# NVIDIA/k8s-cc-manager

Measured on AMD Instinct MI355X. Metric: reconcile_gpus_per_sec, higher is better.
Workload: dtype bf16; 1 GPU; model=cc-mode-transition, global_batch=1, seq_len=1024, parallelism=concurrent-per-gpu x1, modes=on<->off toggle, device_tier=shadow+hip-attest, eviction=True, components=5, attest_gemm_dim=1024

## Files before the change

### k8s_cc_manager_amd/ops/attest_kernels.hip

```cpp

#include <hip/hip_runtime.h>
#include <hip/hip_bf16.h>

#include <cstdint>
#include <cstdio>
#include <cstdlib>
#include <mutex>

#define CC_CHECK(expr)                                                         \
  do {                                                                         \
    hipError_t _e = (expr);                                                    \
    if (_e != hipSuccess) {                                                    \
      snprintf(rep->error, sizeof(rep->error), "%s: %s", #expr,                \
               hipGetErrorString(_e));                                         \
      return (int)_e;                                                          \
    }                                                                          \
  } while (0)

using bf16 = __bf16;
typedef __attribute__((ext_vector_type(8))) bf16 bf16x8;
typedef __attribute__((ext_vector_type(4))) float f32x4;
typedef __attribute__((ext_vector_type(4))) float float4v;

constexpr int BM = 128;
constexpr int BN = 128;
constexpr int BK = 64;

__global__ void fill_bf16_lcg(bf16* __restrict__ out, long n, uint32_t seed) {
  long i = (long)blockIdx.x * blockDim.x + threadIdx.x;
  long stride = (long)gridDim.x * blockDim.x;
  for (; i < n; i += stride) {
    uint32_t x = (uint32_t)i * 1103515245u + seed * 747796405u + 12345u;
    x ^= x >> 16;
    x *= 2654435769u;
    int v = (int)((x >> 13) & 3u) - 2;
    out[i] = (bf16)(float)v;
  }
}

__global__ void fill_fp8_lcg(unsigned char* __restrict__ out, long n,
                             uint32_t seed) {
  const unsigned char enc[4] = {0xC0, 0xB8, 0x00, 0x38};
  long i = (long)blockIdx.x * blockDim.x + threadIdx.x;
  long stride = (long)gridDim.x * blockDim.x;
  for (; i < n; i += stride) {
    uint32_t x = (uint32_t)i * 1103515245u + seed * 747796405u + 12345u;
    x ^= x >> 16;
    x *= 2654435769u;
    out[i] = enc[(x >> 13) & 3u];
  }
}

constexpr int TILE_B = BM * BK * 2;

__device__ __forceinline__ int swz(int byte_off) {
  return byte_off ^ (((byte_off >> 8) & 7) << 4);
}

__device__ __forceinline__ void stage_tile_glds(
    const char* gbase, long row_stride_b, long k0_b, char* lds_tile,
    int wave, int lane) {
#pragma unroll
  for (int p = 0; p < 4; ++p) {
    int base = (wave * 4 + p) * 1024;
// ... 1304 lines not shown
}

__global__ void ref_gemm_f32(const bf16* __restrict__ A,
                             const bf16* __restrict__ Bt,
                             float* __restrict__ C, int M, int N, int K) {
  int col = blockIdx.x * blockDim.x + threadIdx.x;
  int row = blockIdx.y * blockDim.y + threadIdx.y;
  if (row >= M || col >= N) return;
  float acc = 0.f;
  const bf16* a = A + (long)row * K;
  const bf16* b = Bt + (long)col * K;
  for (int k = 0; k < K; ++k) acc = fmaf((float)a[k], (float)b[k], acc);
  C[(long)row * N + col] = acc;
}

__global__ void max_abs_diff(const float* __restrict__ x,
                             const float* __restrict__ y, long n,
                             float* out) {
  __shared__ float smax[256];
  long i = (long)blockIdx.x * blockDim.x + threadIdx.x;
  long stride = (long)gridDim.x * blockDim.x;
  float m = 0.f;
  for (; i < n; i += stride) {
    float d = fabsf(x[i] - y[i]);
    m = fmaxf(m, d);
  }
  smax[threadIdx.x] = m;
  __syncthreads();
  for (int s = 128; s > 0; s >>= 1) {
    if (threadIdx.x < s) smax[threadIdx.x] = fmaxf(smax[threadIdx.x], smax[threadIdx.x + s]);
    __syncthreads();
  }
  if (threadIdx.x == 0) {
    atomicMax((unsigned int*)out, __float_as_uint(smax[0]));
  }
}

__global__ void checksum_f32(const float* __restrict__ x, long n,
                             unsigned long long* out) {
  long i = (long)blockIdx.x * blockDim.x + threadIdx.x;
  long stride = (long)gridDim.x * blockDim.x;
  unsigned long long h = 0;
  for (; i < n; i += stride) {
    unsigned long long v = (unsigned long long)__float_as_uint(x[i]) + 0x9e3779b97f4a7c15ull * (unsigned long long)(i + 1);
    v ^= v >> 33; v *= 0xff51afd7ed558ccdull; v ^= v >> 33;
    h ^= v;
  }
  for (int off = 32; off > 0; off >>= 1)
    h ^= __shfl_down(h, off, 64);
  __shared__ unsigned long long partial[4];
  if ((threadIdx.x & 63) == 0) partial[threadIdx.x >> 6] = h;
  __syncthreads();
  if (threadIdx.x == 0) {
    unsigned long long b = partial[0];
    for (int w = 1; w < (int)(blockDim.x >> 6); ++w) b ^= partial[w];
    atomicXor(out, b);
  }
}

constexpr int LDS_PROBE_WORDS = 16384;

__global__ void lds_probe(uint32_t* __restrict__ fail_count, int rounds) {
  __shared__ uint32_t slab[LDS_PROBE_WORDS];
  const int tid = threadIdx.x;
  const int nthreads = blockDim.x;
  uint32_t local_fail = 0;
  for (int r = 0; r < rounds; ++r) {
    uint32_t salt = 0x9e3779b9u * (r + 1) + blockIdx.x;
    for (int i = tid; i < LDS_PROBE_WORDS; i += nthreads)
      slab[i] = (uint32_t)i * 2654435769u + salt;
    __syncthreads();
    for (int i = tid; i < LDS_PROBE_WORDS; i += nthreads) {
// ... 3 lines not shown
    }
    __syncthreads();
  }
  if (local_fail) atomicAdd(fail_count, local_fail);
}

__global__ void hbm_copy_f4(const float4v* __restrict__ src,
                            float4v* __restrict__ dst, long n4) {
  long i = (long)blockIdx.x * blockDim.x + threadIdx.x;
  long stride = (long)gridDim.x * blockDim.x;
  for (; i < n4; i += stride) dst[i] = src[i];
}

constexpr int kMaxDevices = 64;

struct ProbeCtx {
  int dim = 0;
  int ref_valid = 0;
  bf16 *dA = nullptr, *dB = nullptr;
  unsigned char *dA8 = nullptr, *dB8 = nullptr;
  float *dC = nullptr, *dRef = nullptr, *dHbm = nullptr, *dErr = nullptr;
  unsigned long long* dSum = nullptr;
  uint32_t* dFail = nullptr;
  int* dLive = nullptr;
  hipEvent_t ev0 = nullptr, ev1 = nullptr;
  float* dPeerDst = nullptr;
  long peer_cap = 0;
  unsigned long long* dPeerSum = nullptr;
  int peer_cursor = 0;
};

static ProbeCtx g_ctx[kMaxDevices];
static std::mutex g_ctx_mu;

static void ctx_release(ProbeCtx& c) {
  if (c.dA) (void)hipFree(c.dA);
  if (c.dB) (void)hipFree(c.dB);
  if (c.dA8) (void)hipFree(c.dA8);
  if (c.dB8) (void)hipFree(c.dB8);
  if (c.dC) (void)hipFree(c.dC);
  if (c.dRef) (void)hipFree(c.dRef);
  if (c.dHbm) (void)hipFree(c.dHbm);
  if (c.dErr) (void)hipFree(c.dErr);
  if (c.dSum) (void)hipFree(c.dSum);
  if (c.dFail) (void)hipFree(c.dFail);
  if (c.dLive) (void)hipFree(c.dLive);
  if (c.dPeerDst) (void)hipFree(c.dPeerDst);
  if (c.dPeerSum) (void)hipFree(c.dPeerSum);
  if (c.ev0) (void)hipEventDestroy(c.ev0);
  if (c.ev1) (void)hipEventDestroy(c.ev1);
  c = ProbeCtx{};
}

static hipError_t ctx_acquire(int device, int dim, ProbeCtx** out) {
  ProbeCtx& c = g_ctx[device];
  if (c.dim == dim) {
    *out = &c;
    return hipSuccess;
  }
  ctx_release(c);
  long elems = (long)dim * dim;
  hipError_t e;
  if ((e = hipMalloc(&c.dA, elems * sizeof(bf16))) != hipSuccess) return e;
  if ((e = hipMalloc(&c.dB, elems * sizeof(bf16))) != hipSuccess) return e;
  if ((e = hipMalloc(&c.dA8, elems)) != hipSuccess) return e;
  if ((e = hipMalloc(&c.dB8, elems)) != hipSuccess) return e;
  if ((e = hipMalloc(&c.dC, elems * sizeof(float))) != hipSuccess) return e;
  if ((e = hipMalloc(&c.dRef, elems * sizeof(float))) != hipSuccess) return e;
  if ((e = hipMalloc(&c.dHbm, elems * sizeof(float))) != hipSuccess) return e;
  if ((e = hipMalloc(&c.dErr, sizeof(float))) != hipSuccess) return e;
  if ((e = hipMalloc(&c.dSum, sizeof(unsigned long long))) != hipSuccess) return e;
  if ((e = hipMalloc(&c.dFail, sizeof(uint32_t))) != hipSuccess) return e;
  if ((e = hipMalloc(&c.dLive, sizeof(int))) != hipSuccess) return e;
  if ((e = hipEventCreate(&c.ev0)) != hipSuccess) return e;
  if ((e = hipEventCreate(&c.ev1)) != hipSuccess) return e;
  c.dim = dim;
  *out = &c;
  return hipSuccess;
}


extern "C" {

struct CcAttestReport {
  int device;
  int cu_count;
  int xcc_count;
  char arch[64];
  char error[256];
  long long vram_total_mb;
// ... 15 lines not shown
  int peers_attempted;
  int peers_verified;
  double xgmi_ms;
  double xgmi_gbps_min;
  double xgmi_gbps_max;
  int ok;
};

__global__ void liveness_kernel(int* out) {
  if (threadIdx.x == 0 && blockIdx.x == 0) *out = 0x600D;
}

int cc_device_alive(int device) {
  if (device < 0 || device >= kMaxDevices) return -1;
  if (hipSetDevice(device) != hipSuccess) return -1;
  int* d = nullptr;
  {
    std::lock_guard<std::mutex> lk(g_ctx_mu);
    ProbeCtx& c = g_ctx[device];
    if (!c.dLive && hipMalloc(&c.dLive, sizeof(int)) != hipSuccess) return -2;
    d = c.dLive;
  }
  if (hipMemset(d, 0, sizeof(int)) != hipSuccess) return -2;
  hipLaunchKernelGGL(liveness_kernel, dim3(1), dim3(64), 0, 0, d);
  int h = 0;
  hipError_t e = hipMemcpy(&h, d, sizeof(int), hipMemcpyDeviceToHost);
  if (e != hipSuccess) return -3;
  return h == 0x600D ? 0 : -4;
}

int cc_device_count(void) {
  int n = 0;
  if (hipGetDeviceCount(&n) != hipSuccess) return -1;
  return n;
}

int cc_device_index_for_bdf(int domain, int bus, int dev) {
  int n = 0;
  if (hipGetDeviceCount(&n) != hipSuccess) return -1;
  for (int i = 0; i < n; ++i) {
    hipDeviceProp_t p;
    if (hipGetDeviceProperties(&p, i) != hipSuccess) continue;
    if (p.pciDomainID == domain && p.pciBusID == bus && p.pciDeviceID == dev)
      return i;
  }
  return -1;
}

static int launch_mfma_gemm(const void* A, const void* Bt, void* C, int M,
                            int N, int K) {
  if (M % BM == 0 && N % BN == 0 && K % BK == 0 &&
      ((long)(N / BN) * (M / BM)) <= 256) {
    dim3 grid(N / BN, M / BM);
    hipLaunchKernelGGL(mfma_gemm_bf16, grid, dim3(256), 0, 0, (const bf16*)A,
                       (const bf16*)Bt, (float*)C, M, N, K);
    return 0;
  }
  if (M % BM2 == 0 && N % BN2 == 0 && K % (2 * BK2) == 0) {
    dim3 grid(N / BN2, M / BM2);
    long ws = 2L * K * (M + N) + 4L * M * N;
    int swz_on = ws > (256L << 20) ? 1 : 0;
    if ((long)grid.x * grid.y <= 256)
      hipLaunchKernelGGL(mfma_gemm_bf16_256w, grid, dim3(512), 0, 0,
                         (const bf16*)A, (const bf16*)Bt, (float*)C, M, N, K,
                         swz_on);
    else
      hipLaunchKernelGGL(mfma_gemm_bf16_256, grid, dim3(512), 0, 0,
                         (const bf16*)A, (const bf16*)Bt, (float*)C, M, N, K,
                         swz_on);
    return 0;
  }
  if (M % BM || N % BN || K % BK) return -2;
  dim3 grid(N / BN, M / BM);
  hipLaunchKernelGGL(mfma_gemm_bf16, grid, dim3(256), 0, 0, (const bf16*)A,
                     (const bf16*)Bt, (float*)C, M, N, K);
  return 0;
}

int cc_mfma_gemm_bf16(int device, const void* A, const void* Bt, void* C,
                      int M, int N, int K) {
  if (hipSetDevice(device) != hipSuccess) return -3;
  int rc = launch_mfma_gemm(A, Bt, C, M, N, K);
  if (rc != 0) return rc;
  return (int)hipDeviceSynchronize();
}

int cc_mfma_gemm_bf16_variant(int device, const void* A, const void* Bt,
                              void* C, int M, int N, int K, int which) {
  if (hipSetDevice(device) != hipSuccess) return -3;
// ... 88 lines not shown
    dim3 grid(N / BN2, M / BM2);
    long ws = (long)K * (M + N) + 4L * M * N;
    hipLaunchKernelGGL(mfma_gemm_fp8_256, grid, dim3(512), 0, 0,
                       (const char*)A, (const char*)Bt, (float*)C, M, N, K,
                       ws > (256L << 20) ? 1 : 0);
  } else {
    if (M % BM || N % BN || K % BK8) return -2;
    dim3 grid(N / BN, M / BM);
    hipLaunchKernelGGL(mfma_gemm_fp8_128, grid, dim3(256), 0, 0,
                       (const char*)A, (const char*)Bt, (float*)C, M, N, K);
  }
  return (int)hipDeviceSynchronize();
}

static int launch_fp8_best(const void* A, const void* Bt, void* C, int M,
                           int N, int K) {
  if (M % BM || N % BN) return -2;
  dim3 grid(N / BN, M / BM);
  long ws = (long)K * (M + N) + 4L * M * N;
  int swz_on = ws > (256L << 20) ? 1 : 0;
  if (K % BK8 == 0) {
    long blocks = (long)grid.x * grid.y;
    if (blocks <= 256)
      hipLaunchKernelGGL(mfma_gemm_fp8_128pc, grid, dim3(512), 0, 0,
                         (const char*)A, (const char*)Bt, (float*)C, M, N, K,
                         swz_on);
    else
      hipLaunchKernelGGL(mfma_gemm_fp8_128u, grid, dim3(256), 0, 0,
                         (const char*)A, (const char*)Bt, (float*)C, M, N, K,
                         swz_on);
    return 0;
  }
  if (K % 64 == 0) {
    hipLaunchKernelGGL(mfma_gemm_fp8_128s, grid, dim3(256), 0, 0,
                       (const char*)A, (const char*)Bt, (float*)C, M, N, K);
    return 0;
  }
  return -2;
}

int cc_mfma_gemm_fp8(int device, const void* A, const void* Bt, void* C,
                     int M, int N, int K) {
  if (hipSetDevice(device) != hipSuccess) return -3;
  int rc = launch_fp8_best(A, Bt, C, M, N, K);
  if (rc != 0) return rc;
  return (int)hipDeviceSynchronize();
}

int cc_ref_gemm_f32(int device, const void* A, const void* Bt, void* C,
                    int M, int N, int K) {
  if (hipSetDevice(device) != hipSuccess) return -3;
  dim3 block(16, 16);
  dim3 grid((N + 15) / 16, (M + 15) / 16);
  hipLaunchKernelGGL(ref_gemm_f32, grid, block, 0, 0, (const bf16*)A,
                     (const bf16*)Bt, (float*)C, M, N, K);
  return (int)hipDeviceSynchronize();
}

static double event_ms(hipEvent_t a, hipEvent_t b) {
  float ms = 0.f;
  (void)hipEventElapsedTime(&ms, a, b);
  return (double)ms;
}

int cc_attest_device(int device, int gemm_dim, struct CcAttestReport* rep) {
  if (!rep) return -1;
  __builtin_memset(rep, 0, sizeof(*rep));
  rep->device = device;
  CC_CHECK(hipSetDevice(device));

  hipDeviceProp_t prop;
  CC_CHECK(hipGetDeviceProperties(&prop, device));
  rep->cu_count = prop.multiProcessorCount;
  rep->vram_total_mb = (long long)(prop.totalGlobalMem >> 20);
  __builtin_strncpy(rep->arch, prop.gcnArchName, sizeof(rep->arch) - 1);

  const int D = (gemm_dim / BM) * BM > 0 ? (gemm_dim / BM) * BM : BM;
  rep->gemm_m = rep->gemm_n = rep->gemm_k = D;
  long elems = (long)D * D;

  std::lock_guard<std::mutex> lk(g_ctx_mu);
  if (device < 0 || device >= kMaxDevices) return -5;
  ProbeCtx* ctx = nullptr;
  CC_CHECK(ctx_acquire(device, D, &ctx));
  bf16 *dA = ctx->dA, *dB = ctx->dB;
  float *dC = ctx->dC, *dRef = ctx->dRef, *dErr = ctx->dErr;
  unsigned long long* dSum = ctx->dSum;
  hipEvent_t ev0 = ctx->ev0, ev1 = ctx->ev1;
  CC_CHECK(hipMemset(dErr, 0, sizeof(float)));
  CC_CHECK(hipMemset(dSum, 0, sizeof(unsigned long long)));

  hipLaunchKernelGGL(fill_bf16_lcg, dim3(2048), dim3(256), 0, 0, dA, elems, 1u);
  hipLaunchKernelGGL(fill_bf16_lcg, dim3(2048), dim3(256), 0, 0, dB, elems, 7u);

  launch_mfma_gemm(dA, dB, dC, D, D, D);
  CC_CHECK(hipDeviceSynchronize());
  CC_CHECK(hipEventRecord(ev0, 0));
  launch_mfma_gemm(dA, dB, dC, D, D, D);
  CC_CHECK(hipEventRecord(ev1, 0));
  CC_CHECK(hipEventSynchronize(ev1));
  rep->gemm_ms = event_ms(ev0, ev1);
  rep->gemm_tflops = 2.0 * D * (double)D * D / (rep->gemm_ms * 1e-3) / 1e12;

  if (!ctx->ref_valid) {
    CC_CHECK(hipEventRecord(ev0, 0));
    {
      dim3 rblock(16, 16), rgrid((D + 15) / 16, (D + 15) / 16);
      hipLaunchKernelGGL(ref_gemm_f32, rgrid, rblock, 0, 0, dA, dB, dRef, D, D,
                         D);
    }
    CC_CHECK(hipEventRecord(ev1, 0));
    CC_CHECK(hipEventSynchronize(ev1));
    rep->ref_ms = event_ms(ev0, ev1);
    ctx->ref_valid = 1;
  } else {
    rep->ref_ms = 0.0;
  }

  hipLaunchKernelGGL(max_abs_diff, dim3(1024), dim3(256), 0, 0, dC, dRef,
                     elems, dErr);
  hipLaunchKernelGGL(checksum_f32, dim3(1024), dim3(256), 0, 0, dC, elems, dSum);
  CC_CHECK(hipDeviceSynchronize());
  unsigned int err_bits = 0;
  CC_CHECK(hipMemcpy(&err_bits, dErr, sizeof(err_bits), hipMemcpyDeviceToHost));
  float max_err;
  __builtin_memcpy(&max_err, &err_bits, sizeof(max_err));
  rep->max_abs_err = max_err;
  CC_CHECK(hipMemcpy(&rep->checksum, dSum, sizeof(rep->checksum),
                     hipMemcpyDeviceToHost));

  hipLaunchKernelGGL(fill_fp8_lcg, dim3(2048), dim3(256), 0, 0, ctx->dA8,
                     elems, 1u);
  hipLaunchKernelGGL(fill_fp8_lcg, dim3(2048), dim3(256), 0, 0, ctx->dB8,
                     elems, 7u);
  {
    if (launch_fp8_best(ctx->dA8, ctx->dB8, dC, D, D, D) != 0) return -6;
    CC_CHECK(hipDeviceSynchronize());
    CC_CHECK(hipEventRecord(ev0, 0));
    if (launch_fp8_best(ctx->dA8, ctx->dB8, dC, D, D, D) != 0) return -6;
    CC_CHECK(hipEventRecord(ev1, 0));
    CC_CHECK(hipEventSynchronize(ev1));
    rep->fp8_ms = event_ms(ev0, ev1);
    rep->fp8_tflops = 2.0 * D * (double)D * D / (rep->fp8_ms * 1e-3) / 1e12;
    CC_CHECK(hipMemset(dErr, 0, sizeof(float)));
    hipLaunchKernelGGL(max_abs_diff, dim3(1024), dim3(256), 0, 0, dC, dRef,
                       elems, dErr);
    CC_CHECK(hipDeviceSynchronize());
    unsigned int e8 = 0;
    CC_CHECK(hipMemcpy(&e8, dErr, sizeof(e8), hipMemcpyDeviceToHost));
    float f8err;
    __builtin_memcpy(&f8err, &e8, sizeof(f8err));
    rep->fp8_max_abs_err = f8err;
  }

  uint32_t* dFail = ctx->dFail;
  CC_CHECK(hipMemset(dFail, 0, sizeof(uint32_t)));
  CC_CHECK(hipEventRecord(ev0, 0));
  hipLaunchKernelGGL(lds_probe, dim3(512), dim3(256), 0, 0, dFail, 8);
  CC_CHECK(hipEventRecord(ev1, 0));
  CC_CHECK(hipEventSynchronize(ev1));
  rep->lds_ms = event_ms(ev0, ev1);
  CC_CHECK(hipMemcpy(&rep->lds_failures, dFail, sizeof(uint32_t),
                     hipMemcpyDeviceToHost));

  long n4 = elems / 4;
  CC_CHECK(hipEventRecord(ev0, 0));
  hipLaunchKernelGGL(hbm_copy_f4, dim3(4096), dim3(256), 0, 0,
                     (const float4v*)dC, (float4v*)ctx->dHbm, n4);
  CC_CHECK(hipEventRecord(ev1, 0));
  CC_CHECK(hipEventSynchronize(ev1));
  rep->hbm_ms = event_ms(ev0, ev1);
  rep->hbm_gbps = 2.0 * n4 * 16.0 / (rep->hbm_ms * 1e-3) / 1e9;

  int ndev = 0;
  CC_CHECK(hipGetDeviceCount(&ndev));
  rep->peer_count = ndev - 1;
  if (ndev > kMaxDevices) ndev = kMaxDevices;
  long bytes = elems * sizeof(float);
  if (bytes > (2L << 20)) bytes = 2L << 20;
  long sum_elems = bytes / sizeof(float);
  CC_CHECK(hipMemset(dSum, 0, sizeof(unsigned long long)));
  hipLaunchKernelGGL(checksum_f32, dim3(1024), dim3(256), 0, 0, dC, sum_elems,
                     dSum);
  CC_CHECK(hipDeviceSynchronize());
  unsigned long long src_sum = 0;
  CC_CHECK(hipMemcpy(&src_sum, dSum, sizeof(src_sum), hipMemcpyDeviceToHost));
  int acc[kMaxDevices];
  int n_acc = 0;
  for (int p = 0; p < ndev; ++p) {
    if (p == device) continue;
    int can = 0;
    if (hipDeviceCanAccessPeer(&can, device, p) == hipSuccess && can)
      acc[n_acc++] = p;
  }
  rep->peers_accessible = n_acc;
  int max_peers = 0;
  if (const char* mp = getenv("CC_ATTEST_XGMI_MAX_PEERS")) max_peers = atoi(mp);
  int attempts = (max_peers > 0 && max_peers < n_acc) ? max_peers : n_acc;
  rep->peers_attempted = attempts;
  for (int t = 0; t < attempts; ++t) {
    int p = acc[(ctx->peer_cursor + t) % (n_acc ? n_acc : 1)];
    hipError_t pe = hipDeviceEnablePeerAccess(p, 0);
    if (pe != hipSuccess && pe != hipErrorPeerAccessAlreadyEnabled) {
      (void)hipGetLastError();
    }
    ProbeCtx& pc = g_ctx[p];
    CC_CHECK(hipSetDevice(p));
    if (pc.peer_cap < bytes) {
      if (pc.dPeerDst) (void)hipFree(pc.dPeerDst);
      pc.dPeerDst = nullptr;
      pc.peer_cap = 0;
      if (hipMalloc(&pc.dPeerDst, bytes) != hipSuccess) {
        CC_CHECK(hipSetDevice(device));
        continue;
      }
      pc.peer_cap = bytes;
    }
    if (!pc.dPeerSum &&
        hipMalloc(&pc.dPeerSum, sizeof(unsigned long long)) != hipSuccess) {
      CC_CHECK(hipSetDevice(device));
      continue;
    }
    CC_CHECK(hipMemset(pc.dPeerDst, 0, bytes));
    CC_CHECK(hipSetDevice(device));
    const int kPeerIters = 4;
    CC_CHECK(hipEventRecord(ev0, 0));
    for (int it = 0; it < kPeerIters; ++it)
      CC_CHECK(hipMemcpyPeerAsync(pc.dPeerDst, p, dC, device, bytes, 0));
    CC_CHECK(hipEventRecord(ev1, 0));
    CC_CHECK(hipEventSynchronize(ev1));
    double ms = event_ms(ev0, ev1);
    rep->xgmi_ms += ms;
    double gbps = (double)bytes * kPeerIters / (ms * 1e-3) / 1e9;
    if (rep->xgmi_gbps_min == 0.0 || gbps < rep->xgmi_gbps_min)
      rep->xgmi_gbps_min = gbps;
    if (gbps > rep->xgmi_gbps_max) rep->xgmi_gbps_max = gbps;
    CC_CHECK(hipSetDevice(p));
    CC_CHECK(hipMemset(pc.dPeerSum, 0, sizeof(unsigned long long)));
    hipLaunchKernelGGL(checksum_f32, dim3(1024), dim3(256), 0, 0, pc.dPeerDst,
                       sum_elems, pc.dPeerSum);
    CC_CHECK(hipDeviceSynchronize());
    unsigned long long peer_sum = 0;
    CC_CHECK(hipMemcpy(&peer_sum, pc.dPeerSum, sizeof(peer_sum),
                       hipMemcpyDeviceToHost));
    CC_CHECK(hipSetDevice(device));
    if (peer_sum == src_sum) ++rep->peers_verified;
  }
  if (n_acc) ctx->peer_cursor = (ctx->peer_cursor + attempts) % n_acc;

  rep->ok = (rep->max_abs_err == 0.0f) && (rep->fp8_max_abs_err == 0.0f) &&
                    (rep->lds_failures == 0) && (rep->gemm_tflops > 0.0) &&
                    (rep->peers_verified == rep->peers_attempted)
                ? 1
                : 0;
  return 0;
}

int cc_report_sizeof(void) { return (int)sizeof(struct CcAttestReport); }

void cc_attest_shutdown(void) {
  std::lock_guard<std::mutex> lk(g_ctx_mu);
  for (int i = 0; i < kMaxDevices; ++i) {
    if (g_ctx[i].dim || g_ctx[i].dLive) {
      (void)hipSetDevice(i);
      ctx_release(g_ctx[i]);
    }
  }
}

}
```

Baseline: 318.4 GPU-transitions/s.

## Batch attestation probes on a per-device stream with fused fill and compare kernels

Moves the attestation legs onto a per-device non-blocking stream with per-leg events and one pinned results struct read back once. It replaces the separate blocking memset/launch/memcpy syncs per leg, and caches device properties, peer access lists and the BDF lookup. The bf16 and fp8 fill kernels are fused into one vectorized kernel, and max-abs-diff plus checksum become a single pass. A global mutex is replaced by per-device locks so concurrent GPUs do not serialize. The cost is more complex state handling, and cached facts can go stale if devices change.

```diff
diff --git a/k8s_cc_manager_amd/ops/attest_kernels.hip b/k8s_cc_manager_amd/ops/attest_kernels.hip
--- a/k8s_cc_manager_amd/ops/attest_kernels.hip
+++ b/k8s_cc_manager_amd/ops/attest_kernels.hip
@@ -26,28 +26,54 @@
 constexpr int BN = 128;
 constexpr int BK = 64;
 
-__global__ void fill_bf16_lcg(bf16* __restrict__ out, long n, uint32_t seed) {
-  long i = (long)blockIdx.x * blockDim.x + threadIdx.x;
+struct ProbeResults {
+  uint32_t err_bf16_bits;
+  uint32_t err_fp8_bits;
+  unsigned long long sum_bf16;
+  unsigned long long sum_slice;
+  uint32_t lds_fail;
+  uint32_t pad_;
+};
+
+__device__ __forceinline__ uint32_t lcg_idx(uint32_t i, uint32_t seed) {
+  uint32_t x = i * 1103515245u + seed * 747796405u + 12345u;
+  x ^= x >> 16;
+  x *= 2654435769u;
+  return (x >> 13) & 3u;
+}
+
+__global__ void fill_probe_lcg(uint4* __restrict__ a16, uint4* __restrict__ b16,
+                               uint2* __restrict__ a8, uint2* __restrict__ b8,
+                               long n8, uint32_t seed_a, uint32_t seed_b,
+                               ProbeResults* zero) {
+  const unsigned long long kBf16 = 0x3F800000BF80C000ull;
+  const uint32_t kE4m3 = 0x3800B8C0u;
+  long g = (long)blockIdx.x * blockDim.x + threadIdx.x;
   long stride = (long)gridDim.x * blockDim.x;
-  for (; i < n; i += stride) {
-    uint32_t x = (uint32_t)i * 1103515245u + seed * 747796405u + 12345u;
-    x ^= x >> 16;
-    x *= 2654435769u;
-    int v = (int)((x >> 13) & 3u) - 2;
-    out[i] = (bf16)(float)v;
-  }
-}
-
-__global__ void fill_fp8_lcg(unsigned char* __restrict__ out, long n,
-                             uint32_t seed) {
-  const unsigned char enc[4] = {0xC0, 0xB8, 0x00, 0x38};
-  long i = (long)blockIdx.x * blockDim.x + threadIdx.x;
-  long stride = (long)gridDim.x * blockDim.x;
-  for (; i < n; i += stride) {
-    uint32_t x = (uint32_t)i * 1103515245u + seed * 747796405u + 12345u;
-    x ^= x >> 16;
-    x *= 2654435769u;
-    out[i] = enc[(x >> 13) & 3u];
+  if (zero && g == 0) *zero = ProbeResults{};
+  for (; g < n8; g += stride) {
+    uint32_t base = (uint32_t)(g * 8);
+    uint32_t wa[4], wb[4], ba[2] = {0u, 0u}, bb[2] = {0u, 0u};
+#pragma unroll
+    for (int j = 0; j < 8; ++j) {
+      uint32_t ia = lcg_idx(base + j, seed_a);
+      uint32_t ib = lcg_idx(base + j, seed_b);
+      uint32_t ha = (uint32_t)(kBf16 >> (ia * 16)) & 0xFFFFu;
+      uint32_t hb = (uint32_t)(kBf16 >> (ib * 16)) & 0xFFFFu;
+      if (j & 1) {
+        wa[j >> 1] |= ha << 16;
+        wb[j >> 1] |= hb << 16;
+      } else {
+        wa[j >> 1] = ha;
+        wb[j >> 1] = hb;
+      }
+      ba[j >> 2] |= ((kE4m3 >> (ia * 8)) & 0xFFu) << ((j & 3) * 8);
+      bb[j >> 2] |= ((kE4m3 >> (ib * 8)) & 0xFFu) << ((j & 3) * 8);
+    }
+    a16[g] = make_uint4(wa[0], wa[1], wa[2], wa[3]);
+    b16[g] = make_uint4(wb[0], wb[1], wb[2], wb[3]);
+    a8[g] = make_uint2(ba[0], ba[1]);
+    b8[g] = make_uint2(bb[0], bb[1]);
   }
 }
 
@@ -1382,48 +1408,76 @@
   C[(long)row * N + col] = acc;
 }
 
-__global__ void max_abs_diff(const float* __restrict__ x,
-                             const float* __restrict__ y, long n,
-                             float* out) {
-  __shared__ float smax[256];
-  long i = (long)blockIdx.x * blockDim.x + threadIdx.x;
+__device__ __forceinline__ unsigned long long mix_f32(float x, long i) {
+  unsigned long long v = (unsigned long long)__float_as_uint(x) +
+                         0x9e3779b97f4a7c15ull * (unsigned long long)(i + 1);
+  v ^= v >> 33;
+  v *= 0xff51afd7ed558ccdull;
+  v ^= v >> 33;
+  return v;
+}
+
+template <bool WITH_REF>
+__global__ __launch_bounds__(256) void compare_checksum(
+    const float4v* __restrict__ x, const float4v* __restrict__ ref, long n8,
+    long slice_n, uint32_t* err_out, unsigned long long* sum_out,
+    unsigned long long* slice_out) {
+  long g = (long)blockIdx.x * blockDim.x + threadIdx.x;
   long stride = (long)gridDim.x * blockDim.x;
+  const bool want_slice = slice_out != nullptr;
   float m = 0.f;
-  for (; i < n; i += stride) {
-    float d = fabsf(x[i] - y[i]);
-    m = fmaxf(m, d);
-  }
-  smax[threadIdx.x] = m;
-  __syncthreads();
-  for (int s = 128; s > 0; s >>= 1) {
-    if (threadIdx.x < s) smax[threadIdx.x] = fmaxf(smax[threadIdx.x], smax[threadIdx.x + s]);
-    __syncthreads();
-  }
-  if (threadIdx.x == 0) {
-    atomicMax((unsigned int*)out, __float_as_uint(smax[0]));
-  }
-}
-
-__global__ void checksum_f32(const float* __restrict__ x, long n,
-                             unsigned long long* out) {
-  long i = (long)blockIdx.x * blockDim.x + threadIdx.x;
-  long stride = (long)gridDim.x * blockDim.x;
-  unsigned long long h = 0;
-  for (; i < n; i += stride) {
-    unsigned long long v = (unsigned long long)__float_as_uint(x[i]) + 0x9e3779b97f4a7c15ull * (unsigned long long)(i + 1);
-    v ^= v >> 33; v *= 0xff51afd7ed558ccdull; v ^= v >> 33;
-    h ^= v;
-  }
-  for (int off = 32; off > 0; off >>= 1)
+  unsigned long long h = 0, hs = 0;
+  for (; g < n8; g += stride) {
+    float4v x0 = x[2 * g], x1 = x[2 * g + 1];
+    if (WITH_REF) {
+      float4v r0 = ref[2 * g], r1 = ref[2 * g + 1];
+#pragma unroll
+      for (int j = 0; j < 4; ++j) {
+        m = fmaxf(m, fabsf(x0[j] - r0[j]));
+        m = fmaxf(m, fabsf(x1[j] - r1[j]));
+      }
+    }
+    long i = g * 8;
+#pragma unroll
+    for (int j = 0; j < 8; ++j) {
+      unsigned long long v = mix_f32(j < 4 ? x0[j & 3] : x1[j & 3], i + j);
+      h ^= v;
+      if (want_slice && i + j < slice_n) hs ^= v;
+    }
+  }
+  uint32_t mb = __float_as_uint(m);
+  for (int off = 32; off > 0; off >>= 1) {
     h ^= __shfl_down(h, off, 64);
-  __shared__ unsigned long long partial[4];
-  if ((threadIdx.x & 63) == 0) partial[threadIdx.x >> 6] = h;
+    if (want_slice) hs ^= __shfl_down(hs, off, 64);
+    if (WITH_REF) {
+      uint32_t o = __shfl_down(mb, off, 64);
+      mb = o > mb ? o : mb;
+    }
+  }
+  __shared__ unsigned long long part_h[4], part_s[4];
+  __shared__ uint32_t part_m[4];
+  if ((threadIdx.x & 63) == 0) {
+    part_h[threadIdx.x >> 6] = h;
+    part_s[threadIdx.x >> 6] = hs;
+    part_m[threadIdx.x >> 6] = mb;
+  }
   __syncthreads();
   if (threadIdx.x == 0) {
-    unsigned long long b = partial[0];
-    for (int w = 1; w < (int)(blockDim.x >> 6); ++w) b ^= partial[w];
-    atomicXor(out, b);
-  }
+    for (int w = 1; w < 4; ++w) {
+      part_h[0] ^= part_h[w];
+      part_s[0] ^= part_s[w];
+      part_m[0] = part_m[w] > part_m[0] ? part_m[w] : part_m[0];
+    }
+    if (WITH_REF && err_out) atomicMax(err_out, part_m[0]);
+    if (sum_out) atomicXor(sum_out, part_h[0]);
+    if (want_slice) atomicXor(slice_out, part_s[0]);
+  }
+}
+
+static inline unsigned grid_for_groups(long n8, unsigned cap) {
+  long blocks = (n8 + 255) / 256;
+  if (blocks < 1) blocks = 1;
+  return (unsigned)(blocks < (long)cap ? blocks : (long)cap);
 }
 
 constexpr int LDS_PROBE_WORDS = 16384;
@@ -1457,26 +1511,39 @@
 
 constexpr int kMaxDevices = 64;
 
+enum { LEG_GEMM = 0, LEG_REF, LEG_FP8, LEG_LDS, LEG_HBM, LEG_XGMI, LEG_COUNT };
+
 struct ProbeCtx {
+  std::mutex mu;
+  std::mutex peer_mu;
   int dim = 0;
   int ref_valid = 0;
   bf16 *dA = nullptr, *dB = nullptr;
   unsigned char *dA8 = nullptr, *dB8 = nullptr;
-  float *dC = nullptr, *dRef = nullptr, *dHbm = nullptr, *dErr = nullptr;
-  unsigned long long* dSum = nullptr;
-  uint32_t* dFail = nullptr;
+  float *dC = nullptr, *dRef = nullptr, *dHbm = nullptr;
+  ProbeResults* dRes = nullptr;
+  ProbeResults* hRes = nullptr;
   int* dLive = nullptr;
-  hipEvent_t ev0 = nullptr, ev1 = nullptr;
+  hipStream_t stream = nullptr;
+  hipEvent_t ev[LEG_COUNT][2] = {};
+  int peer_cursor = 0;
+  int facts_valid = 0;
+  int cu_count = 0;
+  long long vram_total_mb = 0;
+  char arch[64] = {};
+  int ndev = 0;
+  int n_acc = 0;
+  int acc[kMaxDevices] = {};
   float* dPeerDst = nullptr;
   long peer_cap = 0;
   unsigned long long* dPeerSum = nullptr;
-  int peer_cursor = 0;
+  hipStream_t peer_stream = nullptr;
 };
 
 static ProbeCtx g_ctx[kMaxDevices];
-static std::mutex g_ctx_mu;
 
 static void ctx_release(ProbeCtx& c) {
+  if (c.stream) (void)hipStreamSynchronize(c.stream);
   if (c.dA) (void)hipFree(c.dA);
   if (c.dB) (void)hipFree(c.dB);
   if (c.dA8) (void)hipFree(c.dA8);
@@ -1484,15 +1551,64 @@
   if (c.dC) (void)hipFree(c.dC);
   if (c.dRef) (void)hipFree(c.dRef);
   if (c.dHbm) (void)hipFree(c.dHbm);
-  if (c.dErr) (void)hipFree(c.dErr);
-  if (c.dSum) (void)hipFree(c.dSum);
-  if (c.dFail) (void)hipFree(c.dFail);
+  if (c.dRes) (void)hipFree(c.dRes);
+  if (c.hRes) (void)hipHostFree(c.hRes);
   if (c.dLive) (void)hipFree(c.dLive);
+  for (int l = 0; l < LEG_COUNT; ++l)
+    for (int k = 0; k < 2; ++k) {
+      if (c.ev[l][k]) (void)hipEventDestroy(c.ev[l][k]);
+      c.ev[l][k] = nullptr;
+    }
+  if (c.stream) (void)hipStreamDestroy(c.stream);
+  c.dA = c.dB = nullptr;
+  c.dA8 = c.dB8 = nullptr;
+  c.dC = c.dRef = c.dHbm = nullptr;
+  c.dRes = c.hRes = nullptr;
+  c.dLive = nullptr;
+  c.stream = nullptr;
+  c.dim = 0;
+  c.ref_valid = 0;
+  c.peer_cursor = 0;
+}
+
+static void ctx_release_peer(ProbeCtx& c) {
+  if (c.peer_stream) (void)hipStreamSynchronize(c.peer_stream);
   if (c.dPeerDst) (void)hipFree(c.dPeerDst);
   if (c.dPeerSum) (void)hipFree(c.dPeerSum);
-  if (c.ev0) (void)hipEventDestroy(c.ev0);
-  if (c.ev1) (void)hipEventDestroy(c.ev1);
-  c = ProbeCtx{};
+  if (c.peer_stream) (void)hipStreamDestroy(c.peer_stream);
+  c.dPeerDst = nullptr;
+  c.dPeerSum = nullptr;
+  c.peer_stream = nullptr;
+  c.peer_cap = 0;
+}
+
+static hipError_t ctx_stream(ProbeCtx& c) {
+  if (c.stream) return hipSuccess;
+  return hipStreamCreateWithFlags(&c.stream, hipStreamNonBlocking);
+}
+
+static hipError_t ctx_facts(ProbeCtx& c, int device) {
+  if (c.facts_valid) return hipSuccess;
+  hipDeviceProp_t prop;
+  hipError_t e;
+  if ((e = hipGetDeviceProperties(&prop, device)) != hipSuccess) return e;
+  c.cu_count = prop.multiProcessorCount;
+  c.vram_total_mb = (long long)(prop.totalGlobalMem >> 20);
+  __builtin_memset(c.arch, 0, sizeof(c.arch));
+  __builtin_strncpy(c.arch, prop.gcnArchName, sizeof(c.arch) - 1);
+  int ndev = 0;
+  if ((e = hipGetDeviceCount(&ndev)) != hipSuccess) return e;
+  c.ndev = ndev;
+  if (ndev > kMaxDevices) ndev = kMaxDevices;
+  c.n_acc = 0;
+  for (int p = 0; p < ndev; ++p) {
+    if (p == device) continue;
+    int can = 0;
+    if (hipDeviceCanAccessPeer(&can, device, p) == hipSuccess && can)
+      c.acc[c.n_acc++] = p;
+  }
+  c.facts_valid = 1;
+  return hipSuccess;
 }
 
 static hipError_t ctx_acquire(int device, int dim, ProbeCtx** out) {
@@ -1504,6 +1620,7 @@
   ctx_release(c);
   long elems = (long)dim * dim;
   hipError_t e;
+  if ((e = ctx_stream(c)) != hipSuccess) return e;
   if ((e = hipMalloc(&c.dA, elems * sizeof(bf16))) != hipSuccess) return e;
   if ((e = hipMalloc(&c.dB, elems * sizeof(bf16))) != hipSuccess) return e;
   if ((e = hipMalloc(&c.dA8, elems)) != hipSuccess) return e;
@@ -1511,12 +1628,12 @@
   if ((e = hipMalloc(&c.dC, elems * sizeof(float))) != hipSuccess) return e;
   if ((e = hipMalloc(&c.dRef, elems * sizeof(float))) != hipSuccess) return e;
   if ((e = hipMalloc(&c.dHbm, elems * sizeof(float))) != hipSuccess) return e;
-  if ((e = hipMalloc(&c.dErr, sizeof(float))) != hipSuccess) return e;
-  if ((e = hipMalloc(&c.dSum, sizeof(unsigned long long))) != hipSuccess) return e;
-  if ((e = hipMalloc(&c.dFail, sizeof(uint32_t))) != hipSuccess) return e;
+  if ((e = hipMalloc(&c.dRes, sizeof(ProbeResults))) != hipSuccess) return e;
+  if ((e = hipHostMalloc(&c.hRes, sizeof(ProbeResults))) != hipSuccess) return e;
   if ((e = hipMalloc(&c.dLive, sizeof(int))) != hipSuccess) return e;
-  if ((e = hipEventCreate(&c.ev0)) != hipSuccess) return e;
-  if ((e = hipEventCreate(&c.ev1)) != hipSuccess) return e;
+  for (int l = 0; l < LEG_COUNT; ++l)
+    for (int k = 0; k < 2; ++k)
+      if ((e = hipEventCreate(&c.ev[l][k])) != hipSuccess) return e;
   c.dim = dim;
   *out = &c;
   return hipSuccess;
@@ -1562,17 +1679,15 @@
 int cc_device_alive(int device) {
   if (device < 0 || device >= kMaxDevices) return -1;
   if (hipSetDevice(device) != hipSuccess) return -1;
-  int* d = nullptr;
-  {
-    std::lock_guard<std::mutex> lk(g_ctx_mu);
-    ProbeCtx& c = g_ctx[device];
-    if (!c.dLive && hipMalloc(&c.dLive, sizeof(int)) != hipSuccess) return -2;
-    d = c.dLive;
-  }
-  if (hipMemset(d, 0, sizeof(int)) != hipSuccess) return -2;
-  hipLaunchKernelGGL(liveness_kernel, dim3(1), dim3(64), 0, 0, d);
+  ProbeCtx& c = g_ctx[device];
+  std::lock_guard<std::mutex> lk(c.mu);
+  if (ctx_stream(c) != hipSuccess) return -2;
+  if (!c.dLive && hipMalloc(&c.dLive, sizeof(int)) != hipSuccess) return -2;
+  if (hipMemsetAsync(c.dLive, 0, sizeof(int), c.stream) != hipSuccess) return -2;
+  hipLaunchKernelGGL(liveness_kernel, dim3(1), dim3(64), 0, c.stream, c.dLive);
   int h = 0;
-  hipError_t e = hipMemcpy(&h, d, sizeof(int), hipMemcpyDeviceToHost);
+  hipError_t e = hipMemcpyWithStream(&h, c.dLive, sizeof(int),
+                                     hipMemcpyDeviceToHost, c.stream);
   if (e != hipSuccess) return -3;
   return h == 0x600D ? 0 : -4;
 }
@@ -1583,24 +1698,38 @@
   return n;
 }
 
+static std::mutex g_bdf_mu;
+static int g_bdf_n = -1;
+static int g_bdf[kMaxDevices][3];
+
 int cc_device_index_for_bdf(int domain, int bus, int dev) {
-  int n = 0;
-  if (hipGetDeviceCount(&n) != hipSuccess) return -1;
-  for (int i = 0; i < n; ++i) {
-    hipDeviceProp_t p;
-    if (hipGetDeviceProperties(&p, i) != hipSuccess) continue;
-    if (p.pciDomainID == domain && p.pciBusID == bus && p.pciDeviceID == dev)
+  std::lock_guard<std::mutex> lk(g_bdf_mu);
+  if (g_bdf_n < 0) {
+    int n = 0;
+    if (hipGetDeviceCount(&n) != hipSuccess) return -1;
+    if (n > kMaxDevices) n = kMaxDevices;
+    for (int i = 0; i < n; ++i) {
+      hipDeviceProp_t p;
+      g_bdf[i][0] = g_bdf[i][1] = g_bdf[i][2] = -1;
+      if (hipGetDeviceProperties(&p, i) != hipSuccess) continue;
+      g_bdf[i][0] = p.pciDomainID;
+      g_bdf[i][1] = p.pciBusID;
+      g_bdf[i][2] = p.pciDeviceID;
+    }
+    g_bdf_n = n;
+  }
+  for (int i = 0; i < g_bdf_n; ++i)
+    if (g_bdf[i][0] == domain && g_bdf[i][1] == bus && g_bdf[i][2] == dev)
       return i;
-  }
   return -1;
 }
 
 static int launch_mfma_gemm(const void* A, const void* Bt, void* C, int M,
-                            int N, int K) {
+                            int N, int K, hipStream_t stream = 0) {
   if (M % BM == 0 && N % BN == 0 && K % BK == 0 &&
       ((long)(N / BN) * (M / BM)) <= 256) {
     dim3 grid(N / BN, M / BM);
-    hipLaunchKernelGGL(mfma_gemm_bf16, grid, dim3(256), 0, 0, (const bf16*)A,
+    hipLaunchKernelGGL(mfma_gemm_bf16, grid, dim3(256), 0, stream, (const bf16*)A,
                        (const bf16*)Bt, (float*)C, M, N, K);
     return 0;
   }
@@ -1609,18 +1738,18 @@
     long ws = 2L * K * (M + N) + 4L * M * N;
     int swz_on = ws > (256L << 20) ? 1 : 0;
     if ((long)grid.x * grid.y <= 256)
-      hipLaunchKernelGGL(mfma_gemm_bf16_256w, grid, dim3(512), 0, 0,
+      hipLaunchKernelGGL(mfma_gemm_bf16_256w, grid, dim3(512), 0, stream,
                          (const bf16*)A, (const bf16*)Bt, (float*)C, M, N, K,
                          swz_on);
     else
-      hipLaunchKernelGGL(mfma_gemm_bf16_256, grid, dim3(512), 0, 0,
+      hipLaunchKernelGGL(mfma_gemm_bf16_256, grid, dim3(512), 0, stream,
                          (const bf16*)A, (const bf16*)Bt, (float*)C, M, N, K,
                          swz_on);
     return 0;
   }
   if (M % BM || N % BN || K % BK) return -2;
   dim3 grid(N / BN, M / BM);
-  hipLaunchKernelGGL(mfma_gemm_bf16, grid, dim3(256), 0, 0, (const bf16*)A,
+  hipLaunchKernelGGL(mfma_gemm_bf16, grid, dim3(256), 0, stream, (const bf16*)A,
                      (const bf16*)Bt, (float*)C, M, N, K);
   return 0;
 }
@@ -1739,7 +1868,7 @@
 }
 
 static int launch_fp8_best(const void* A, const void* Bt, void* C, int M,
-                           int N, int K) {
+                           int N, int K, hipStream_t stream = 0) {
   if (M % BM || N % BN) return -2;
   dim3 grid(N / BN, M / BM);
   long ws = (long)K * (M + N) + 4L * M * N;
@@ -1747,17 +1876,17 @@
   if (K % BK8 == 0) {
     long blocks = (long)grid.x * grid.y;
     if (blocks <= 256)
-      hipLaunchKernelGGL(mfma_gemm_fp8_128pc, grid, dim3(512), 0, 0,
+      hipLaunchKernelGGL(mfma_gemm_fp8_128pc, grid, dim3(512), 0, stream,
                          (const char*)A, (const char*)Bt, (float*)C, M, N, K,
                          swz_on);
     else
-      hipLaunchKernelGGL(mfma_gemm_fp8_128u, grid, dim3(256), 0, 0,
+      hipLaunchKernelGGL(mfma_gemm_fp8_128u, grid, dim3(256), 0, stream,
                          (const char*)A, (const char*)Bt, (float*)C, M, N, K,
                          swz_on);
     return 0;
   }
   if (K % 64 == 0) {
-    hipLaunchKernelGGL(mfma_gemm_fp8_128s, grid, dim3(256), 0, 0,
+    hipLaunchKernelGGL(mfma_gemm_fp8_128s, grid, dim3(256), 0, stream,
                        (const char*)A, (const char*)Bt, (float*)C, M, N, K);
     return 0;
   }
@@ -1788,187 +1917,194 @@
   return (double)ms;
 }
 
+#define CC_CHECK_Q(expr)                                                       \
+  do {                                                                         \
+    hipError_t _e = (expr);                                                    \
+    if (_e != hipSuccess) {                                                    \
+      snprintf(rep->error, sizeof(rep->error), "%s: %s", #expr,                \
+               hipGetErrorString(_e));                                         \
+      (void)hipStreamSynchronize(q);                                           \
+      return (int)_e;                                                          \
+    }                                                                          \
+  } while (0)
+
+#define CC_CHECK_P(expr)                                                       \
+  do {                                                                         \
+    hipError_t _e = (expr);                                                    \
+    if (_e != hipSuccess) {                                                    \
+      snprintf(rep->error, sizeof(rep->error), "%s: %s", #expr,                \
+               hipGetErrorString(_e));                                         \
+      if (pc.peer_stream) (void)hipStreamSynchronize(pc.peer_stream);          \
+      (void)hipStreamSynchronize(q);                                           \
+      (void)hipSetDevice(device);                                              \
+      return (int)_e;                                                          \
+    }                                                                          \
+  } while (0)
+
 int cc_attest_device(int device, int gemm_dim, struct CcAttestReport* rep) {
   if (!rep) return -1;
   __builtin_memset(rep, 0, sizeof(*rep));
   rep->device = device;
   CC_CHECK(hipSetDevice(device));
-
-  hipDeviceProp_t prop;
-  CC_CHECK(hipGetDeviceProperties(&prop, device));
-  rep->cu_count = prop.multiProcessorCount;
-  rep->vram_total_mb = (long long)(prop.totalGlobalMem >> 20);
-  __builtin_strncpy(rep->arch, prop.gcnArchName, sizeof(rep->arch) - 1);
+  if (device < 0 || device >= kMaxDevices) return -5;
+
+  std::lock_guard<std::mutex> lk(g_ctx[device].mu);
+  CC_CHECK(ctx_facts(g_ctx[device], device));
+  rep->cu_count = g_ctx[device].cu_count;
+  rep->vram_total_mb = g_ctx[device].vram_total_mb;
+  __builtin_memcpy(rep->arch, g_ctx[device].arch, sizeof(rep->arch));
 
   const int D = (gemm_dim / BM) * BM > 0 ? (gemm_dim / BM) * BM : BM;
   rep->gemm_m = rep->gemm_n = rep->gemm_k = D;
   long elems = (long)D * D;
 
-  std::lock_guard<std::mutex> lk(g_ctx_mu);
-  if (device < 0 || device >= kMaxDevices) return -5;
   ProbeCtx* ctx = nullptr;
   CC_CHECK(ctx_acquire(device, D, &ctx));
   bf16 *dA = ctx->dA, *dB = ctx->dB;
-  float *dC = ctx->dC, *dRef = ctx->dRef, *dErr = ctx->dErr;
-  unsigned long long* dSum = ctx->dSum;
-  hipEvent_t ev0 = ctx->ev0, ev1 = ctx->ev1;
-  CC_CHECK(hipMemset(dErr, 0, sizeof(float)));
-  CC_CHECK(hipMemset(dSum, 0, sizeof(unsigned long long)));
-
-  hipLaunchKernelGGL(fill_bf16_lcg, dim3(2048), dim3(256), 0, 0, dA, elems, 1u);
-  hipLaunchKernelGGL(fill_bf16_lcg, dim3(2048), dim3(256), 0, 0, dB, elems, 7u);
-
-  launch_mfma_gemm(dA, dB, dC, D, D, D);
-  CC_CHECK(hipDeviceSynchronize());
-  CC_CHECK(hipEventRecord(ev0, 0));
-  launch_mfma_gemm(dA, dB, dC, D, D, D);
-  CC_CHECK(hipEventRecord(ev1, 0));
-  CC_CHECK(hipEventSynchronize(ev1));
-  rep->gemm_ms = event_ms(ev0, ev1);
+  float *dC = ctx->dC, *dRef = ctx->dRef;
+  ProbeResults* dRes = ctx->dRes;
+  hipStream_t q = ctx->stream;
+  hipEvent_t(*ev)[2] = ctx->ev;
+
+  const int n_acc = ctx->n_acc;
+  rep->peer_count = ctx->ndev - 1;
+  rep->peers_accessible = n_acc;
+  int max_peers = 0;
+  if (const char* mp = getenv("CC_ATTEST_XGMI_MAX_PEERS")) max_peers = atoi(mp);
+  const int attempts = (max_peers > 0 && max_peers < n_acc) ? max_peers : n_acc;
+  rep->peers_attempted = attempts;
+  long bytes = elems * sizeof(float);
+  if (bytes > (2L << 20)) bytes = 2L << 20;
+  const long sum_elems = bytes / sizeof(float);
+
+  const bool cold = !ctx->ref_valid;
+
+  const long n8 = elems / 8;
+  hipLaunchKernelGGL(fill_probe_lcg, dim3(grid_for_groups(n8, 2048)), dim3(256),
+                     0, q, (uint4*)dA, (uint4*)dB, (uint2*)ctx->dA8,
+                     (uint2*)ctx->dB8, n8, 1u, 7u, dRes);
+
+  if (cold) launch_mfma_gemm(dA, dB, dC, D, D, D, q);
+  CC_CHECK_Q(hipEventRecord(ev[LEG_GEMM][0], q));
+  launch_mfma_gemm(dA, dB, dC, D, D, D, q);
+  CC_CHECK_Q(hipEventRecord(ev[LEG_GEMM][1], q));
+
+  if (cold) {
+    CC_CHECK_Q(hipEventRecord(ev[LEG_REF][0], q));
+    dim3 rblock(16, 16), rgrid((D + 15) / 16, (D + 15) / 16);
+    hipLaunchKernelGGL(ref_gemm_f32, rgrid, rblock, 0, q, dA, dB, dRef, D, D, D);
+    CC_CHECK_Q(hipEventRecord(ev[LEG_REF][1], q));
+  }
+
+  const unsigned cgrid = grid_for_groups(n8, 512);
+  hipLaunchKernelGGL(compare_checksum<true>, dim3(cgrid), dim3(256), 0, q,
+                     (const float4v*)dC, (const float4v*)dRef, n8, 0L,
+                     &dRes->err_bf16_bits, &dRes->sum_bf16,
+                     (unsigned long long*)nullptr);
+
+  if (cold && launch_fp8_best(ctx->dA8, ctx->dB8, dC, D, D, D, q) != 0) {
+    (void)hipStreamSynchronize(q);
+    return -6;
+  }
+  CC_CHECK_Q(hipEventRecord(ev[LEG_FP8][0], q));
+  if (launch_fp8_best(ctx->dA8, ctx->dB8, dC, D, D, D, q) != 0) {
+    (void)hipStreamSynchronize(q);
+    return -6;
+  }
+  CC_CHECK_Q(hipEventRecord(ev[LEG_FP8][1], q));
+  hipLaunchKernelGGL(compare_checksum<true>, dim3(cgrid), dim3(256), 0, q,
+                     (const float4v*)dC, (const float4v*)dRef, n8, sum_elems,
+                     &dRes->err_fp8_bits, (unsigned long long*)nullptr,
+                     attempts > 0 ? &dRes->sum_slice : nullptr);
+
+  CC_CHECK_Q(hipEventRecord(ev[LEG_LDS][0], q));
+  hipLaunchKernelGGL(lds_probe, dim3(512), dim3(256), 0, q, &dRes->lds_fail, 8);
+  CC_CHECK_Q(hipEventRecord(ev[LEG_LDS][1], q));
+
+  long n4 = elems / 4;
+  CC_CHECK_Q(hipEventRecord(ev[LEG_HBM][0], q));
+  hipLaunchKernelGGL(hbm_copy_f4, dim3(4096), dim3(256), 0, q,
+                     (const float4v*)dC, (float4v*)ctx->dHbm, n4);
+  CC_CHECK_Q(hipEventRecord(ev[LEG_HBM][1], q));
+
+  CC_CHECK_Q(hipMemcpyAsync(ctx->hRes, dRes, sizeof(ProbeResults),
+                            hipMemcpyDeviceToHost, q));
+  CC_CHECK(hipStreamSynchronize(q));
+
+  const ProbeResults res = *ctx->hRes;
+  rep->gemm_ms = event_ms(ev[LEG_GEMM][0], ev[LEG_GEMM][1]);
   rep->gemm_tflops = 2.0 * D * (double)D * D / (rep->gemm_ms * 1e-3) / 1e12;
-
-  if (!ctx->ref_valid) {
-    CC_CHECK(hipEventRecord(ev0, 0));
-    {
-      dim3 rblock(16, 16), rgrid((D + 15) / 16, (D + 15) / 16);
-      hipLaunchKernelGGL(ref_gemm_f32, rgrid, rblock, 0, 0, dA, dB, dRef, D, D,
-                         D);
-    }
-    CC_CHECK(hipEventRecord(ev1, 0));
-    CC_CHECK(hipEventSynchronize(ev1));
-    rep->ref_ms = event_ms(ev0, ev1);
+  if (cold) {
+    rep->ref_ms = event_ms(ev[LEG_REF][0], ev[LEG_REF][1]);
     ctx->ref_valid = 1;
   } else {
     rep->ref_ms = 0.0;
   }
-
-  hipLaunchKernelGGL(max_abs_diff, dim3(1024), dim3(256), 0, 0, dC, dRef,
-                     elems, dErr);
-  hipLaunchKernelGGL(checksum_f32, dim3(1024), dim3(256), 0, 0, dC, elems, dSum);
-  CC_CHECK(hipDeviceSynchronize());
-  unsigned int err_bits = 0;
-  CC_CHECK(hipMemcpy(&err_bits, dErr, sizeof(err_bits), hipMemcpyDeviceToHost));
-  float max_err;
-  __builtin_memcpy(&max_err, &err_bits, sizeof(max_err));
-  rep->max_abs_err = max_err;
-  CC_CHECK(hipMemcpy(&rep->checksum, dSum, sizeof(rep->checksum),
-                     hipMemcpyDeviceToHost));
-
-  hipLaunchKernelGGL(fill_fp8_lcg, dim3(2048), dim3(256), 0, 0, ctx->dA8,
-                     elems, 1u);
-  hipLaunchKernelGGL(fill_fp8_lcg, dim3(2048), dim3(256), 0, 0, ctx->dB8,
-                     elems, 7u);
-  {
-    if (launch_fp8_best(ctx->dA8, ctx->dB8, dC, D, D, D) != 0) return -6;
-    CC_CHECK(hipDeviceSynchronize());
-    CC_CHECK(hipEventRecord(ev0, 0));
-    if (launch_fp8_best(ctx->dA8, ctx->dB8, dC, D, D, D) != 0) return -6;
-    CC_CHECK(hipEventRecord(ev1, 0));
-    CC_CHECK(hipEventSynchronize(ev1));
-    rep->fp8_ms = event_ms(ev0, ev1);
-    rep->fp8_tflops = 2.0 * D * (double)D * D / (rep->fp8_ms * 1e-3) / 1e12;
-    CC_CHECK(hipMemset(dErr, 0, sizeof(float)));
-    hipLaunchKernelGGL(max_abs_diff, dim3(1024), dim3(256), 0, 0, dC, dRef,
-                       elems, dErr);
-    CC_CHECK(hipDeviceSynchronize());
-    unsigned int e8 = 0;
-    CC_CHECK(hipMemcpy(&e8, dErr, sizeof(e8), hipMemcpyDeviceToHost));
-    float f8err;
-    __builtin_memcpy(&f8err, &e8, sizeof(f8err));
-    rep->fp8_max_abs_err = f8err;
-  }
-
-  uint32_t* dFail = ctx->dFail;
-  CC_CHECK(hipMemset(dFail, 0, sizeof(uint32_t)));
-  CC_CHECK(hipEventRecord(ev0, 0));
-  hipLaunchKernelGGL(lds_probe, dim3(512), dim3(256), 0, 0, dFail, 8);
-  CC_CHECK(hipEventRecord(ev1, 0));
-  CC_CHECK(hipEventSynchronize(ev1));
-  rep->lds_ms = event_ms(ev0, ev1);
-  CC_CHECK(hipMemcpy(&rep->lds_failures, dFail, sizeof(uint32_t),
-                     hipMemcpyDeviceToHost));
-
-  long n4 = elems / 4;
-  CC_CHECK(hipEventRecord(ev0, 0));
-  hipLaunchKernelGGL(hbm_copy_f4, dim3(4096), dim3(256), 0, 0,
-                     (const float4v*)dC, (float4v*)ctx->dHbm, n4);
-  CC_CHECK(hipEventRecord(ev1, 0));
-  CC_CHECK(hipEventSynchronize(ev1));
-  rep->hbm_ms = event_ms(ev0, ev1);
+  __builtin_memcpy(&rep->max_abs_err, &res.err_bf16_bits, sizeof(float));
+  rep->checksum = res.sum_bf16;
+  rep->fp8_ms = event_ms(ev[LEG_FP8][0], ev[LEG_FP8][1]);
+  rep->fp8_tflops = 2.0 * D * (double)D * D / (rep->fp8_ms * 1e-3) / 1e12;
+  __builtin_memcpy(&rep->fp8_max_abs_err, &res.err_fp8_bits, sizeof(float));
+  rep->lds_ms = event_ms(ev[LEG_LDS][0], ev[LEG_LDS][1]);
+  rep->lds_failures = res.lds_fail;
+  rep->hbm_ms = event_ms(ev[LEG_HBM][0], ev[LEG_HBM][1]);
   rep->hbm_gbps = 2.0 * n4 * 16.0 / (rep->hbm_ms * 1e-3) / 1e9;
 
-  int ndev = 0;
-  CC_CHECK(hipGetDeviceCount(&ndev));
-  rep->peer_count = ndev - 1;
-  if (ndev > kMaxDevices) ndev = kMaxDevices;
-  long bytes = elems * sizeof(float);
-  if (bytes > (2L << 20)) bytes = 2L << 20;
-  long sum_elems = bytes / sizeof(float);
-  CC_CHECK(hipMemset(dSum, 0, sizeof(unsigned long long)));
-  hipLaunchKernelGGL(checksum_f32, dim3(1024), dim3(256), 0, 0, dC, sum_elems,
-                     dSum);
-  CC_CHECK(hipDeviceSynchronize());
-  unsigned long long src_sum = 0;
-  CC_CHECK(hipMemcpy(&src_sum, dSum, sizeof(src_sum), hipMemcpyDeviceToHost));
-  int acc[kMaxDevices];
-  int n_acc = 0;
-  for (int p = 0; p < ndev; ++p) {
-    if (p == device) continue;
-    int can = 0;
-    if (hipDeviceCanAccessPeer(&can, device, p) == hipSuccess && can)
-      acc[n_acc++] = p;
-  }
-  rep->peers_accessible = n_acc;
-  int max_peers = 0;
-  if (const char* mp = getenv("CC_ATTEST_XGMI_MAX_PEERS")) max_peers = atoi(mp);
-  int attempts = (max_peers > 0 && max_peers < n_acc) ? max_peers : n_acc;
-  rep->peers_attempted = attempts;
+  const unsigned long long src_sum = res.sum_slice;
   for (int t = 0; t < attempts; ++t) {
-    int p = acc[(ctx->peer_cursor + t) % (n_acc ? n_acc : 1)];
+    int p = ctx->acc[(ctx->peer_cursor + t) % (n_acc ? n_acc : 1)];
     hipError_t pe = hipDeviceEnablePeerAccess(p, 0);
     if (pe != hipSuccess && pe != hipErrorPeerAccessAlreadyEnabled) {
       (void)hipGetLastError();
     }
     ProbeCtx& pc = g_ctx[p];
-    CC_CHECK(hipSetDevice(p));
+    std::lock_guard<std::mutex> plk(pc.peer_mu);
+    CC_CHECK_P(hipSetDevice(p));
+    if (!pc.peer_stream)
+      CC_CHECK_P(hipStreamCreateWithFlags(&pc.peer_stream, hipStreamNonBlocking));
     if (pc.peer_cap < bytes) {
       if (pc.dPeerDst) (void)hipFree(pc.dPeerDst);
       pc.dPeerDst = nullptr;
       pc.peer_cap = 0;
       if (hipMalloc(&pc.dPeerDst, bytes) != hipSuccess) {
-        CC_CHECK(hipSetDevice(device));
+        CC_CHECK_P(hipSetDevice(device));
         continue;
       }
       pc.peer_cap = bytes;
     }
     if (!pc.dPeerSum &&
         hipMalloc(&pc.dPeerSum, sizeof(unsigned long long)) != hipSuccess) {
-      CC_CHECK(hipSetDevice(device));
+      CC_CHECK_P(hipSetDevice(device));
       continue;
     }
-    CC_CHECK(hipMemset(pc.dPeerDst, 0, bytes));
-    CC_CHECK(hipSetDevice(device));
+    CC_CHECK_P(hipMemsetAsync(pc.dPeerDst, 0, bytes, pc.peer_stream));
+    CC_CHECK_P(hipMemsetAsync(pc.dPeerSum, 0, sizeof(unsigned long long),
+                              pc.peer_stream));
+    CC_CHECK_P(hipStreamSynchronize(pc.peer_stream));
+    CC_CHECK_P(hipSetDevice(device));
     const int kPeerIters = 4;
-    CC_CHECK(hipEventRecord(ev0, 0));
+    CC_CHECK_P(hipEventRecord(ev[LEG_XGMI][0], q));
     for (int it = 0; it < kPeerIters; ++it)
-      CC_CHECK(hipMemcpyPeerAsync(pc.dPeerDst, p, dC, device, bytes, 0));
-    CC_CHECK(hipEventRecord(ev1, 0));
-    CC_CHECK(hipEventSynchronize(ev1));
-    double ms = event_ms(ev0, ev1);
+      CC_CHECK_P(hipMemcpyPeerAsync(pc.dPeerDst, p, dC, device, bytes, q));
+    CC_CHECK_P(hipEventRecord(ev[LEG_XGMI][1], q));
+    CC_CHECK_P(hipEventSynchronize(ev[LEG_XGMI][1]));
+    double ms = event_ms(ev[LEG_XGMI][0], ev[LEG_XGMI][1]);
     rep->xgmi_ms += ms;
     double gbps = (double)bytes * kPeerIters / (ms * 1e-3) / 1e9;
     if (rep->xgmi_gbps_min == 0.0 || gbps < rep->xgmi_gbps_min)
       rep->xgmi_gbps_min = gbps;
     if (gbps > rep->xgmi_gbps_max) rep->xgmi_gbps_max = gbps;
-    CC_CHECK(hipSetDevice(p));
-    CC_CHECK(hipMemset(pc.dPeerSum, 0, sizeof(unsigned long long)));
-    hipLaunchKernelGGL(checksum_f32, dim3(1024), dim3(256), 0, 0, pc.dPeerDst,
-                       sum_elems, pc.dPeerSum);
-    CC_CHECK(hipDeviceSynchronize());
+    CC_CHECK_P(hipSetDevice(p));
+    hipLaunchKernelGGL(compare_checksum<false>,
+                       dim3(grid_for_groups(sum_elems / 8, 512)), dim3(256), 0,
+                       pc.peer_stream, (const float4v*)pc.dPeerDst,
+                       (const float4v*)nullptr, sum_elems / 8, 0L,
+                       (uint32_t*)nullptr, pc.dPeerSum,
+                       (unsigned long long*)nullptr);
     unsigned long long peer_sum = 0;
-    CC_CHECK(hipMemcpy(&peer_sum, pc.dPeerSum, sizeof(peer_sum),
-                       hipMemcpyDeviceToHost));
-    CC_CHECK(hipSetDevice(device));
+    CC_CHECK_P(hipMemcpyWithStream(&peer_sum, pc.dPeerSum, sizeof(peer_sum),
+                                   hipMemcpyDeviceToHost, pc.peer_stream));
+    CC_CHECK_P(hipSetDevice(device));
     if (peer_sum == src_sum) ++rep->peers_verified;
   }
   if (n_acc) ctx->peer_cursor = (ctx->peer_cursor + attempts) % n_acc;
@@ -1981,16 +2117,63 @@
   return 0;
 }
 
+#undef CC_CHECK_P
+#undef CC_CHECK_Q
+
+int cc_probe_fill(int device, void* a, void* b, void* a8, void* b8, long n) {
+  if (n <= 0 || n % 8 != 0) return -2;
+  if (((uintptr_t)a | (uintptr_t)b) & 15u) return -2;
+  if (((uintptr_t)a8 | (uintptr_t)b8) & 7u) return -2;
+  if (hipSetDevice(device) != hipSuccess) return -3;
+  hipLaunchKernelGGL(fill_probe_lcg, dim3(grid_for_groups(n / 8, 2048)),
+                     dim3(256), 0, 0, (uint4*)a, (uint4*)b, (uint2*)a8,
+                     (uint2*)b8, n / 8, 1u, 7u, (ProbeResults*)nullptr);
+  return (int)hipStreamSynchronize(0);
+}
+
+int cc_probe_compare(int device, const void* c, const void* ref, long n,
+                     long slice_n, float* err_out,
+                     unsigned long long* sum_out,
+                     unsigned long long* slice_sum_out) {
+  if (n <= 0 || n % 8 != 0) return -2;
+  if (((uintptr_t)c | (uintptr_t)ref) & 15u) return -2;
+  if (slice_n < 0 || slice_n > n) return -2;
+  if (hipSetDevice(device) != hipSuccess) return -3;
+  ProbeResults* d = nullptr;
+  if (hipMalloc(&d, sizeof(ProbeResults)) != hipSuccess) return -4;
+  ProbeResults h{};
+  hipError_t e = hipMemsetAsync(d, 0, sizeof(ProbeResults), 0);
+  if (e == hipSuccess) {
+    hipLaunchKernelGGL(compare_checksum<true>,
+                       dim3(grid_for_groups(n / 8, 512)), dim3(256), 0, 0,
+                       (const float4v*)c, (const float4v*)ref, n / 8, slice_n,
+                       &d->err_bf16_bits, &d->sum_bf16,
+                       slice_sum_out ? &d->sum_slice : nullptr);
+    e = hipMemcpyWithStream(&h, d, sizeof(h), hipMemcpyDeviceToHost, 0);
+  }
+  (void)hipFree(d);
+  if (e != hipSuccess) return (int)e;
+  if (err_out) __builtin_memcpy(err_out, &h.err_bf16_bits, sizeof(float));
+  if (sum_out) *sum_out = h.sum_bf16;
+  if (slice_sum_out) *slice_sum_out = h.sum_slice;
+  return 0;
+}
+
 int cc_report_sizeof(void) { return (int)sizeof(struct CcAttestReport); }
 
 void cc_attest_shutdown(void) {
-  std::lock_guard<std::mutex> lk(g_ctx_mu);
   for (int i = 0; i < kMaxDevices; ++i) {
-    if (g_ctx[i].dim || g_ctx[i].dLive) {
+    ProbeCtx& c = g_ctx[i];
+    std::lock_guard<std::mutex> lk(c.mu);
+    std::lock_guard<std::mutex> plk(c.peer_mu);
+    if (c.dim || c.dLive || c.stream || c.dPeerDst || c.dPeerSum ||
+        c.peer_stream) {
       (void)hipSetDevice(i);
-      ctx_release(g_ctx[i]);
-    }
-  }
-}
-
-}
+      ctx_release(c);
+      ctx_release_peer(c);
+    }
+    c.facts_valid = 0;
+  }
+}
+
+}
```

Result: slower. 288.5 GPU-transitions/s (-9.4%).
